# freshman97/LinTransUNet

Hardware: AMD Instinct MI355X
Metric: 128^3 CT patches/sec (fwd+bwd) (higher is better)
Workload: dtype bf16; 1 GPU; MaskTransUnet train step (fwd + 5-level loss + bwd), 128^3 single-channel patches, 2 per GPU, dropout 0.3, random-init weights; global_batch=2, parallelism=dp1, side_stream_concurrent=True, allreduce=none (1 rank)

## Files before the change

include/ltu_hip.h:

```cpp
#ifndef LTU_HIP_H
#define LTU_HIP_H

#include <stdint.h>

#ifdef __cplusplus
extern "C" {
#endif

typedef void* ltu_stream_t;

enum { LTU_F32 = 0, LTU_BF16 = 1 };
enum { LTU_OK = 0, LTU_E_DTYPE = -1, LTU_E_SHAPE = -2, LTU_E_ALIGN = -3, LTU_E_ARG = -4,
       LTU_E_COMM = -100  };
enum { LTU_ACT_NONE = 0, LTU_ACT_LRELU = 1 };

int ltu_version(void);
int ltu_build_flags(void);
int ltu_config_set(const char* name, int value, int clear);
int ltu_selftest_group_reduce(const float* x, float* sum, float* mx, int n, int G, ltu_stream_t s);
#ifdef LTU_EXPERIMENTS
int ltu_selftest_last_arriver(const float* x, float* part, float* out, unsigned* counter, float* sink, int nwg, int n,
                              int rows_per_chunk, int skew, int mode, ltu_stream_t s);
#endif

int ltu_window_embed(const float* x, void* y, int dtype, int B, int H, int W, int D, ltu_stream_t s);

int ltu_pack_conv_weight(const float* w, void* wf, void* wd, int Co, int Ci, int CoP, int CiP, int out_dtype, ltu_stream_t s);
int ltu_unpack_conv_wgrad(const float* dwf, float* dw, int Co, int Ci, int CiP, ltu_stream_t s);
int ltu_transpose_f32(const float* in, void* out, int R, int C, int ldo, int col_off, int out_dtype, ltu_stream_t s);
int ltu_cast_f32(const float* in, void* out, long long n, int out_dtype, ltu_stream_t s);
int ltu_weight_prep(const void* table, int n, int out_dtype, ltu_stream_t s);
#define LTU_WPREP_CHUNK 4096
int ltu_weight_prep_chunks(const void* table, const int* chunks, int nchunks, int out_dtype, ltu_stream_t s);

int ltu_linear_fwd(const void* a, int lda, const void* const* w, int nw, const float* const* bias, void* y, int ldy,
                   int M, int N, int K, int accumulate, int dtype, ltu_stream_t s);
int ltu_linear_gelu_fwd(const void* a, int lda, const void* w, const float* bias, void* u, void* h, int M, int N, int K, float p,
                        uint64_t seed, const uint64_t* step, int dtype, ltu_stream_t s);
int ltu_layer_tail_fwd(const void* a, const void* x, const void* wo, const void* w1, const void* w2, const float* bo,
                       const float* b1, const float* b2, const float* g1, const float* be1, const float* g2, const float* be2,
                       void* z1, void* t1, void* u, void* h, void* z2, void* y, float* stat1, float* stat2, long long M, int d,
                       float eps, float p, uint64_t seed1, uint64_t seedg, uint64_t seed2, const uint64_t* step, int u_mode,
                       const void* qkv, const float* ctx, float* qstat, int ntok, const void* wq_next, const float* bq0,
                       const float* bq1, const float* bq2, void* qkv_next, int dtype, ltu_stream_t s);

long long ltu_layer_tail_blocks(long long M);
int ltu_layer_tail_bwd(const void* dy, const void* dy2, const void* z2, const void* z1, const void* u, const float* stat2,
                       const float* stat1, const float* g2, const float* g1, const void* w2t, const void* w1t, const void* wot,
                       void* dr2, void* du, void* dr1, void* dz1, void* da, float* lnws2, float* lnws1, long long lnws_floats ,
                       long long M, int d, float p,
                       uint64_t seed1, uint64_t seedg, uint64_t seed2, const uint64_t* step, int u_mode, int dtype, ltu_stream_t s);

typedef struct ltu_reduce_job {
  const float* part;
  int nsplit, n, k, nseg;
  float* out[3];
  float* outb[3];
  int mode;
} ltu_reduce_job;
int ltu_reduce_batch(const ltu_reduce_job* jobs, int njobs, ltu_stream_t s);

long long ltu_wgrad_ws_floats(long long M, int N, int K);
int ltu_linear_wgrad(const void* g, int ldg, const void* a, int lda, float* const* dw, float* const* db, int nw, int M, int N,
                     int K, float* ws, long long ws_floats, ltu_reduce_job* defer, int dtype, ltu_stream_t s);
#define LTU_WGRAD_GROUP_MAX 32
typedef struct ltu_wgrad_job {
  const void* grad;
  const void* a;
  float* dw[3];
  float* db[3];
  int ldg, lda, nw, M, N, K;
} ltu_wgrad_job;
long long ltu_linear_wgrad_group_ws_floats(const ltu_wgrad_job* jobs, int njobs, int blocks);
int ltu_linear_wgrad_group(const ltu_wgrad_job* jobs, int njobs, int blocks, float* ws, long long ws_floats, int dtype, ltu_stream_t s);

long long ltu_upconv_wgrad_ws_floats(long long M, int Co, int Ci, int blocks);

int ltu_conv3d_fwd(const void* x0, const void* x1, const void* wf, const float* bias, void* y, int B, int Hi, int Wi,
                   int Di, int C0, int C1, int Co, int sh, int sw, int sd, int ups, float* ws, long long ws_floats, int dtype,
                   ltu_stream_t s);
long long ltu_conv3d_ws_floats(int B, int H, int W, int D, int C, int Co);
long long ltu_igemm_ws_floats(long long M, int N, int K);
int ltu_conv3d_pair_fwd(const void* x, const void* wf, const float* bias, void* y0, void* y1, int B, int H, int W, int D, int C,
                        int N0, int N1, float* ws, long long ws_floats, int dtype, ltu_stream_t s);
// ... 194 lines not shown
```

lintransunet_amd/_lib.py:

```python
import ctypes
import os
from ctypes import c_float, c_int, c_longlong, c_uint64, c_void_p

_HERE = os.path.dirname(os.path.abspath(__file__))
LIB_PATH = os.path.join(_HERE, os.environ.get('LTU_LIB', 'libltu_hip.so'))

P, I, L, F, U = c_void_p, c_int, c_longlong, c_float, c_uint64


class ReduceJob(ctypes.Structure):
    _fields_ = [('part', c_void_p), ('nsplit', c_int), ('n', c_int), ('k', c_int), ('nseg', c_int),
                ('out', c_void_p * 3), ('outb', c_void_p * 3), ('mode', c_int)]


class WgradJob(ctypes.Structure):
    _fields_ = [('grad', c_void_p), ('a', c_void_p), ('dw', c_void_p * 3), ('db', c_void_p * 3),
                ('ldg', c_int), ('lda', c_int), ('nw', c_int), ('M', c_int), ('N', c_int), ('K', c_int)]


WGRAD_GROUP_MAX = 32
CROP_ORIENT_MAX = 64
BLEND_ITEMS_MAX = 32
U8, I16 = 2, 3


SIGNATURES = {
    'ltu_version': [],
    'ltu_build_flags': [],
    'ltu_config_set': [ctypes.c_char_p, I, I],
    'ltu_selftest_group_reduce': [P, P, P, I, I, P],
    'ltu_window_embed': [P, P, I, I, I, I, I, P],
    'ltu_pack_conv_weight': [P, P, P, I, I, I, I, I, P],
    'ltu_unpack_conv_wgrad': [P, P, I, I, I, P],
    'ltu_transpose_f32': [P, P, I, I, I, I, I, P],
    'ltu_cast_f32': [P, P, L, I, P],
    'ltu_linear_fwd': [P, I, P, I, P, P, I, I, I, I, I, I, P],
    'ltu_wgrad_ws_floats': [L, I, I],
    'ltu_upconv_wgrad_ws_floats': [L, I, I, I],
    'ltu_linear_wgrad': [P, I, P, I, P, P, I, I, I, I, P, L, P, I, P],
    'ltu_layer_tail_fwd': [P, P, P, P, P, P, P, P, P, P, P, P, P, P, P, P, P, P, P, P, L, I, F, F, U, U, U, P, I, P, P, P, I, P, P, P, P, P, I, P],
    'ltu_layer_tail_blocks': [L],
    'ltu_layer_tail_bwd': [P, P, P, P, P, P, P, P, P, P, P, P, P, P, P, P, P, P, P, L, L, I, F, U, U, U, P, I, I, P],
    'ltu_reduce_batch': [P, I, P],
    'ltu_linear_wgrad_group_ws_floats': [P, I, I],
    'ltu_linear_wgrad_group': [P, I, I, P, L, I, P],
    'ltu_conv3d_fwd': [P, P, P, P, P, I, I, I, I, I, I, I, I, I, I, I, P, L, I, P],
    'ltu_conv3d_ws_floats': [I, I, I, I, I, I],
    'ltu_conv3d_pair_fwd': [P, P, P, P, P, I, I, I, I, I, I, I, P, L, I, P],
    'ltu_conv3d_pair_dgrad': [P, P, P, P, I, I, I, I, I, I, I, P, L, I, P],
    'ltu_conv3d_pair_wgrad': [P, P, P, P, P, P, P, I, I, I, I, I, I, I, I, I, I, P, L, I, P],
    'ltu_conv3d_dgrad': [P, P, P, P, I, I, I, I, I, I, I, I, I, I, P, L, I, P],
    'ltu_conv3d_wgrad': [P, P, P, P, P, I, I, I, I, I, I, I, I, I, I, I, I, I, P, L, I, P],
    'ltu_affine_sample': [P, P, P, I, I, I, I, P],
    'ltu_zoom_sample': [P, P, P, I, I, I, I, P],
    'ltu_adjust_contrast': [P, P, P, P, I, L, P],
    'ltu_linear_gelu_fwd': [P, I, P, P, P, P, I, I, I, F, U, P, I, P],
    'ltu_weight_prep': [P, I, I, P],
    'ltu_weight_prep_chunks': [P, P, I, I, P],
    'ltu_sumpool2': [P, P, I, I, I, I, I, I, P],
    'ltu_upconv_fwd': [P, P, P, P, I, I, I, I, I, I, I, P],
    'ltu_upconv_dgrad': [P, P, P, I, I, I, I, I, I, P, L, I, P],
    'ltu_igemm_ws_floats': [L, I, I],
    'ltu_upconv_wgrad': [P, P, P, P, P, I, I, P, L, I, I, I, I, I, I, I, I, P],
    'ltu_linattn_splits': [I, I],
    'ltu_linattn_ws_floats': [I, I, I],
    'ltu_linattn_fwd': [P, P, P, P, P, P, L, I, I, I, I, P],
    'ltu_linattn_ctx': [P, P, P, P, L, I, I, I, I, P],
    'ltu_linattn_bwd': [P, P, P, P, P, P, P, P, P, L, I, I, I, I, P],
    'ltu_window_gather': [P, P, P, I, I, I, I, I, I, I, I, I, I, P],
    'ltu_vote_accumulate': [P, P, P, P, I, I, I, I, I, I, I, I, P],
    'ltu_vote_finalize': [P, P, P, I, I, I, I, I, I, I, I, I, I, I, P],
    'ltu_window_gather_mirror': [P, P, P, I, I, I, I, I, I, I, I, I, I, I, P],
    'ltu_window_blend': [P, P, P, P, P, P, F, P, I, I, I, I, I, I, I, I, I, P],
    'ltu_keep_largest_component': [P, P, P, P, P, I, I, I, I, I, P],
    'ltu_seg_metrics': [P, P, P, P, I, I, I, I, L, F, P],
# ... 119 lines not shown
```

lintransunet_amd/csrc/misc.hip:

```cpp
#include <math.h>

#include "common.h"

#include <mutex>
#include <stdlib.h>

extern "C" int ltu_version(void) { return 4; }
extern "C" int ltu_build_flags(void) {
#ifdef LTU_EXPERIMENTS
  return 1;
#else
  return 0;
#endif
}

template <int G>
__global__ void selftest_reduce_kernel(const float* __restrict__ x, float* __restrict__ sum, float* __restrict__ mx, int n) {
  const int i = blockIdx.x * blockDim.x + threadIdx.x;
  const float v = i < n ? x[i] : 0.f;
  const float s = group_reduce<G, LtuAdd>(v), m = group_reduce<G, LtuMax>(v);
  if (i < n) { sum[i] = s; mx[i] = m; }
}
extern "C" int ltu_selftest_group_reduce(const float* x, float* sum, float* mx, int n, int G, ltu_stream_t s) {
  if (n <= 0 || n % 64) return LTU_E_SHAPE;
// ... 125 lines not shown
    const unsigned dr = stride % R, dc = stride / R;
    for (unsigned i = t0; i < t1; i += stride) {
      st1<TW>(dst + (size_t)c * d.p0 + d.p1 + r, d.src[(size_t)r * C + c]);
      r += dr; c += dc;
      if (r >= R) { r -= R; ++c; }
    }
  } else if (d.kind == 5 || d.kind == 6) {
    const unsigned CoP = (unsigned)d.p0, CiP = (unsigned)d.p1;
    const unsigned n = 64u * CoP * CiP;
    if (t1 > n) t1 = n;
    for (unsigned i = t0; i < t1; i += stride) {
      unsigned cls, sl, co, ci;
      if (d.kind == 5) { ci = i % CiP; const unsigned q = i / CiP; sl = q & 7; co = (q >> 3) % CoP; cls = (q >> 3) / CoP; }
      else { co = i % CoP; const unsigned q = i / CoP; const unsigned cs = q & 63; ci = q >> 6; cls = cs >> 3; sl = cs & 7; }
      float v = 0.f;
      if (co < (unsigned)d.R && ci < (unsigned)d.C) {
        int lo[3], hi[3];
        for (int a = 0; a < 3; ++a) {
          const int p = (cls >> (2 - a)) & 1, sa = (sl >> (2 - a)) & 1;
          if (p == 0) { lo[a] = sa == 0 ? 0 : 1; hi[a] = sa == 0 ? 0 : 2; }
          else { lo[a] = sa == 0 ? 0 : 2; hi[a] = sa == 0 ? 1 : 2; }
        }
        const float* w = d.src + ((size_t)co * d.C + ci) * 27;
        for (int th = lo[0]; th <= hi[0]; ++th)
          for (int tw = lo[1]; tw <= hi[1]; ++tw)
            for (int td = lo[2]; td <= hi[2]; ++td) v += w[(th * 3 + tw) * 3 + td];
      }
      st1<TW>(dst + i, v);
    }
  } else if (d.kind == 8 || d.kind == 9) {
    const unsigned n = (unsigned)d.R * (unsigned)d.C;
    if (t1 > n) t1 = n;
    const unsigned KS = (d.kind == 8 ? (unsigned)d.C : (unsigned)d.R) >> 4;
    for (unsigned i = t0; i < t1; i += stride) {
      const unsigned j = i & 7u, l = (i >> 3) & 63u, t = i >> 9;
      const unsigned ks = t % KS, ct = t / KS;
      const unsigned o = ct * 32u + (l & 31u), r = ks * 16u + 8u * (l >> 5) + j;
      const float v = d.kind == 8 ? d.src[(size_t)o * d.C + r] : d.src[(size_t)r * d.C + o];
      st1<TW>(dst + i, v);
    }
  } else if (d.kind == 7) {
    const unsigned stride_c = (unsigned)d.p0, CiP = (unsigned)d.p1, off = (unsigned)d.pad >> 16, cnt = (unsigned)d.pad & 0xffffu;
    const unsigned n = cnt * 27u * CiP;
    if (t1 > n) t1 = n;
    for (unsigned i = t0; i < t1; i += stride) {
      const unsigned co = i % cnt, q = i / cnt, t = q % 27u, ci = q / 27u;
      const float v = (co < (unsigned)d.R && ci < (unsigned)d.C) ? d.src[((size_t)co * d.C + ci) * 27 + t] : 0.f;
      st1<TW>(dst + ((size_t)ci * 27 + t) * stride_c + off + co, v);
    }
  } else {
    const unsigned CoP = (unsigned)d.p0, CiP = (unsigned)d.p1;
    const unsigned n = CoP * 27u * CiP;
    if (t1 > n) t1 = n;
    const unsigned R0 = d.kind == 2 ? CiP : CoP;
    unsigned x0 = t0 % R0, q = t0 / R0, x1 = q % 27u, x2 = q / 27u;
    const unsigned s0 = stride % R0, sq = stride / R0, s1 = sq % 27u, s2 = sq / 27u;
    for (unsigned i = t0; i < t1; i += stride) {
      const unsigned co = d.kind == 2 ? x2 : x0, ci = d.kind == 2 ? x0 : x2;
      const float v = (co < (unsigned)d.R && ci < (unsigned)d.C) ? d.src[((size_t)co * d.C + ci) * 27 + x1] : 0.f;
      st1<TW>(dst + i, v);
      x0 += s0; x1 += s1; x2 += s2;
      if (x0 >= R0) { x0 -= R0; ++x1; }
      if (x1 >= 27u) { x1 -= 27u; ++x2; }
    }
  }
}

template <typename TW>
__global__ void weight_prep_kernel(const WPrep* __restrict__ table) {
  const WPrep d = table[blockIdx.y];
  weight_prep_range<TW>(d, blockIdx.x * blockDim.x + threadIdx.x, 0x7fffffffu, gridDim.x * blockDim.x);
}
// ... 6 lines not shown
  return true;
}
__device__ __forceinline__ size_t wp8_load(const WPrep& d, unsigned i, float (&f)[8]) {
  const unsigned R = (unsigned)d.R, C = (unsigned)d.C;
  const bool src16 = (reinterpret_cast<uintptr_t>(d.src) & 15) == 0;
  size_t o = i;
  if (d.kind == 0) {
    if (src16) {
      const float4 a = *reinterpret_cast<const float4*>(d.src + i), b = *reinterpret_cast<const float4*>(d.src + i + 4);
      f[0] = a.x; f[1] = a.y; f[2] = a.z; f[3] = a.w; f[4] = b.x; f[5] = b.y; f[6] = b.z; f[7] = b.w;
    } else {
#pragma unroll
      for (int j = 0; j < 8; ++j) f[j] = d.src[i + j];
    }
  } else if (d.kind == 1) {
    const unsigned c = i / R, r = i - c * R;
#pragma unroll
    for (int j = 0; j < 8; ++j) f[j] = d.src[(size_t)(r + j) * C + c];
    o = (size_t)c * d.p0 + d.p1 + r;
  } else {
    const unsigned KS = (d.kind == 8 ? C : R) >> 4;
    const unsigned l = (i >> 3) & 63u, t = i >> 9;
    const unsigned ks = t % KS, ct = t / KS;
    const unsigned oo = ct * 32u + (l & 31u), r = ks * 16u + 8u * (l >> 5);
    if (d.kind == 8 && src16 && C % 4 == 0) {
      const float4 a = *reinterpret_cast<const float4*>(d.src + (size_t)oo * C + r), b = *reinterpret_cast<const float4*>(d.src + (size_t)oo * C + r + 4);
      f[0] = a.x; f[1] = a.y; f[2] = a.z; f[3] = a.w; f[4] = b.x; f[5] = b.y; f[6] = b.z; f[7] = b.w;
    } else if (d.kind == 8) {
#pragma unroll
      for (int j = 0; j < 8; ++j) f[j] = d.src[(size_t)oo * C + r + j];
    } else {
#pragma unroll
      for (int j = 0; j < 8; ++j) f[j] = d.src[(size_t)(r + j) * C + oo];
    }
  }
  return o;
}

template <typename TW, int WP_NC>
__global__ void __launch_bounds__(256) weight_prep_chunk_kernel(const WPrep* __restrict__ table, const int2* __restrict__ chunks, int nchunks) {
  constexpr int PER = LTU_WPREP_CHUNK / 8 / 256;
  static_assert(PER * 256 * 8 == LTU_WPREP_CHUNK, "chunk size");
  for (int c0 = blockIdx.x * WP_NC; c0 < nchunks; c0 += gridDim.x * WP_NC) {
    float f[WP_NC][PER][8];
    uint16_t* dp[WP_NC][PER];
#pragma unroll
    for (int k = 0; k < WP_NC; ++k) {
#pragma unroll
      for (int u = 0; u < PER; ++u) dp[k][u] = nullptr;
      if (c0 + k >= nchunks) continue;
      const int2 c = chunks[c0 + k];
      const WPrep d = table[c.x];
      const unsigned t0 = (unsigned)c.y * LTU_WPREP_CHUNK;
      if (!wp8_ok(d, (int)sizeof(TW))) {
        weight_prep_range<TW>(d, t0 + threadIdx.x, t0 + LTU_WPREP_CHUNK, blockDim.x);
        continue;
      }
      const unsigned n = (unsigned)d.R * (unsigned)d.C;
#pragma unroll
      for (int u = 0; u < PER; ++u) {
        const unsigned i = t0 + (threadIdx.x + u * 256u) * 8u;
        if (i < n) dp[k][u] = reinterpret_cast<uint16_t*>(d.dst) + wp8_load(d, i, f[k][u]);
      }
    }
#pragma unroll
    for (int k = 0; k < WP_NC; ++k)
// ... 74 lines not shown
```

lintransunet_amd/csrc/tlayer.hip:

```cpp
#include "common.h"

#define TL_ROWS 32
#ifndef TL_QDEPTH
#define TL_QDEPTH 8
#endif

struct TailArgs {
  const uint16_t* a;
  const uint16_t* x;
  const uint16_t* wo;
  const uint16_t* w1;
  const uint16_t* w2;
  const float* bo;
  const float* b1;
  const float* b2;
  const float* g1;
  const float* be1;
  const float* g2;
  const float* be2;
  uint16_t* z1;
  uint16_t* t1;
  uint16_t* u;
  uint16_t* h;
  uint16_t* z2;
// ... 348 lines not shown
    for (int i = tid; i < TL_ROWS * CPRQ; i += NTHR) {
      const int r = i / CPRQ, c = (i % CPRQ) * 8;
      if (row0 + r < ta.M) *reinterpret_cast<uint4*>(ta.qkv_next + (row0 + r) * (3 * D) + c) = *reinterpret_cast<const uint4*>(QB + r * LDQ + c);
    }
  }
}

struct TailBwdArgs {
  const uint16_t* dy;
  const uint16_t* dy2;
  const uint16_t* z2;
  const uint16_t* z1;
  const uint16_t* u;
  const float* stat2;
  const float* stat1;
  const float* g2;
  const float* g1;
  const uint16_t* w2t;
  const uint16_t* w1t;
  const uint16_t* wot;
  uint16_t* dr2;
  uint16_t* du;
  uint16_t* dr1;
  uint16_t* dz1;
  uint16_t* da;
  float* lnws2;
  float* lnws1;
  long long M;
  float p;
  uint64_t seed1, seedg, seed2;
  const uint64_t* step;
  int u_mode;
};

template <int D, int NTHR, bool G_LDS, bool G2_LDS, bool DZ_LDS, bool DZ_GLOBAL>
__device__ __forceinline__ void tl_layernorm_bwd(const uint16_t* gl_, const uint16_t* gl2_, const uint16_t* gg1, const uint16_t* gg2,
                                                 const uint16_t* __restrict__ zg, const float* __restrict__ stat,
                                                 const float* __restrict__ gamma, uint16_t* dzl, uint16_t* dzg, uint16_t* drl,
                                                 uint16_t* drg, float* __restrict__ lnws, float* red, int LD, long long row0,
                                                 long long M, const DropCfg& dc, int tid) {
  constexpr int E = D == 128 ? TL_LN_E128 : TL_LN_E256, Q = E / 4;
  constexpr int G = D / E, RPP = NTHR / G, NR = TL_ROWS / RPP;
  const int gl = tid % G, rgp = tid / G;
  float gmv[E], ag[E], ab[E];
#pragma unroll
  for (int q = 0; q < Q; ++q) {
    const float4 t = *reinterpret_cast<const float4*>(gamma + gl * E + 4 * q);
    gmv[4 * q] = t.x; gmv[4 * q + 1] = t.y; gmv[4 * q + 2] = t.z; gmv[4 * q + 3] = t.w;
  }
#pragma unroll
  for (int k = 0; k < E; ++k) { ag[k] = 0.f; ab[k] = 0.f; }
  uint2 zq[NR][Q], q1[NR][Q], q2[NR][Q];
  float2 st[NR];
#pragma unroll
  for (int i = 0; i < NR; ++i) {
    const long long row = row0 + rgp + i * RPP;
#pragma unroll
    for (int q = 0; q < Q; ++q) zq[i][q] = q1[i][q] = q2[i][q] = make_uint2(0u, 0u);
    st[i] = make_float2(0.f, 0.f);
    if (row < M) {
      ld_quads<Q>(zg + row * D + gl * E, zq[i]);
      if (gg1 != nullptr) ld_quads<Q>(gg1 + row * D + gl * E, q1[i]);
      if (gg2 != nullptr) ld_quads<Q>(gg2 + row * D + gl * E, q2[i]);
      st[i] = *reinterpret_cast<const float2*>(stat + row * 2);
    }
  }
// ... 30 lines not shown
      if (ok) { ab[k] += gv[k]; ag[k] += gv[k] * h[k]; }
      gg[k] = gv[k] * gmv[k];
      s1 += gg[k]; s2 += gg[k] * h[k];
    }
    const float m1 = group_sum<G>(s1) / (float)D, m2 = group_sum<G>(s2) / (float)D;
    uint2 dzq[Q], drq[Q];
#pragma unroll
    for (int q = 0; q < Q; ++q) {
      const float4 dz = make_float4(rstd * (gg[4 * q] - m1 - h[4 * q] * m2), rstd * (gg[4 * q + 1] - m1 - h[4 * q + 1] * m2),
                                    rstd * (gg[4 * q + 2] - m1 - h[4 * q + 2] * m2), rstd * (gg[4 * q + 3] - m1 - h[4 * q + 3] * m2));
      dzq[q] = pack_quad(dz.x, dz.y, dz.z, dz.w);
      const float4 dr = drop4(dc, (unsigned long long)(((row * D + gl * E) >> 2) + q), dz);
      drq[q] = pack_quad(dr.x, dr.y, dr.z, dr.w);
    }
    if constexpr (DZ_LDS) st_quads<Q>(dzl + r * LD + gl * E, dzq);
    st_quads<Q>(drl + r * LD + gl * E, drq);
    if (ok) {
      if constexpr (DZ_GLOBAL) st_quads<Q>(dzg + row * D + gl * E, dzq);
      st_quads<Q>(drg + row * D + gl * E, drq);
    }
  }
  float* dst = red + ((long long)rgp * D + gl * E) * 2;
#pragma unroll
  for (int k = 0; k < E; ++k) { dst[2 * k] = ag[k]; dst[2 * k + 1] = ab[k]; }
  __syncthreads();
  for (int i = tid; i < 2 * D; i += NTHR) {
    float acc = 0.f;
#pragma unroll
    for (int q = 0; q < RPP; ++q) acc += red[(long long)q * 2 * D + i];
    lnws[(long long)blockIdx.x * 2 * D + i] = acc;
  }
}

template <int D, int UMODE, int WPS, bool PRE_U>
__global__ void __launch_bounds__(D >= 256 ? 512 : 256, WPS) tail_bwd_kernel(const TailBwdArgs ta) {
  constexpr int LD = D + 8, LDH = 2 * D + 8;
  constexpr int NW = D >= 256 ? 8 : 4, NTHR = NW * 64;
  constexpr int NT1 = D / 32, NT2 = 2 * D / 32;
  static_assert(NT1 == NW && NT2 == 2 * NW, "one d-wide tile and two 2d-wide tiles per wave");
  constexpr int KS1 = D / 16, KS2 = 2 * D / 16;
  extern __shared__ __attribute__((aligned(16))) uint16_t smem[];
  uint16_t* RB = smem;
  uint16_t* ZB = RB + TL_ROWS * LD;
  uint16_t* UB = ZB + TL_ROWS * LD;
  float* red = reinterpret_cast<float*>(UB);
  static_assert((NTHR / (D / (D == 128 ? TL_LN_E128 : TL_LN_E256))) * 2 * D * sizeof(float) <= TL_ROWS * LDH * sizeof(uint16_t), "column-sum scratch fits in UB");
  const int tid = threadIdx.x, lane = tid & 63, wave = tid >> 6;
  const int li = lane & 31, lh = lane >> 5;
  const long long row0 = (long long)blockIdx.x * TL_ROWS;
  const DropCfg dc1 = make_drop(ta.p, ta.seed1, ta.step), dcg = make_drop(ta.p, ta.seedg, ta.step), dc2 = make_drop(ta.p, ta.seed2, ta.step);

  TlQueue<KS1> q1;
  TlQueue<KS2> q2;
  tl_layernorm_bwd<D, NTHR, false, false, true, false>(nullptr, nullptr, ta.dy, ta.dy2, ta.z2, ta.stat2, ta.g2, ZB, nullptr, RB, ta.dr2,
                                                      ta.lnws2, red, LD, row0, ta.M, dc2, tid);
  tl_issue<KS1>(ta.w2t, wave, lane, q1);
  constexpr int CPR2 = 2 * D / 8, NCH2 = TL_ROWS * CPR2 / NTHR;
  uint4 uch[PRE_U ? NCH2 : 1];
  if constexpr (PRE_U) {
#pragma unroll
    for (int j = 0; j < NCH2; ++j) {
      const int i = tid + j * NTHR, r = i / CPR2, c = (i % CPR2) * 8;
      uch[j] = make_uint4(0u, 0u, 0u, 0u);
      if (row0 + r < ta.M) uch[j] = *reinterpret_cast<const uint4*>(ta.u + (row0 + r) * (2 * D) + c);
    }
  }
  __builtin_amdgcn_sched_barrier(0);
  __syncthreads();
  f32x16 acc;
#pragma unroll
  for (int t = 0; t < 2; ++t) {
    const int ct = wave + t * NW;
    tl_run<KS1>(ta.w2t, ct, RB, LD, lane, q1, acc);
    if (t == 0) tl_issue<KS1>(ta.w2t, wave + NW, lane, q1);
    else tl_issue<KS2>(ta.w1t, wave, lane, q2);
#pragma unroll
    for (int q = 0; q < 4; ++q) {
      const int n = ct * 32 + 8 * q + 4 * lh;
      *reinterpret_cast<uint2*>(UB + li * LDH + n) = pack_quad(acc[4 * q], acc[4 * q + 1], acc[4 * q + 2], acc[4 * q + 3]);
    }
  }
  __syncthreads();
#pragma unroll
  for (int j = 0; j < NCH2; ++j) {
    const int i = tid + j * NTHR, r = i / CPR2, c = (i % CPR2) * 8;
    const long long rw = row0 + r;
    const uint4 dv = *reinterpret_cast<const uint4*>(UB + r * LDH + c);
    const float4 d0 = unpack_quad(make_uint2(dv.x, dv.y)), d1 = unpack_quad(make_uint2(dv.z, dv.w));
// ... 15 lines not shown
    }
    const uint4 dq = make_uint4(a0.x, a0.y, a1.x, a1.y);
    *reinterpret_cast<uint4*>(UB + r * LDH + c) = dq;
    if (rw < ta.M) *reinterpret_cast<uint4*>(ta.du + rw * (2 * D) + c) = dq;
  }
  __syncthreads();
  tl_run<KS2>(ta.w1t, wave, UB, LDH, lane, q2, acc);
  tl_issue<KS1>(ta.wot, wave, lane, q1);
#pragma unroll
  for (int q = 0; q < 4; ++q) {
    const int n = wave * 32 + 8 * q + 4 * lh;
    *reinterpret_cast<uint2*>(RB + li * LD + n) = pack_quad(acc[4 * q], acc[4 * q + 1], acc[4 * q + 2], acc[4 * q + 3]);
  }
  __syncthreads();
  tl_layernorm_bwd<D, NTHR, true, true, false, true>(RB, ZB, nullptr, nullptr, ta.z1, ta.stat1, ta.g1, nullptr, ta.dz1, RB, ta.dr1, ta.lnws1,
                                                    red, LD, row0, ta.M, dc1, tid);
  __syncthreads();
  tl_run<KS1>(ta.wot, wave, RB, LD, lane, q1, acc);
#pragma unroll
  for (int q = 0; q < 4; ++q) {
    const int n = wave * 32 + 8 * q + 4 * lh;
    *reinterpret_cast<uint2*>(ZB + li * LD + n) = pack_quad(acc[4 * q], acc[4 * q + 1], acc[4 * q + 2], acc[4 * q + 3]);
  }
  __syncthreads();
  {
    constexpr int CPR = D / 8;
    for (int i = tid; i < TL_ROWS * CPR; i += NTHR) {
      const int r = i / CPR, c = (i % CPR) * 8;
      if (row0 + r < ta.M) *reinterpret_cast<uint4*>(ta.da + (row0 + r) * D + c) = *reinterpret_cast<const uint4*>(ZB + r * LD + c);
    }
  }
}

extern "C" long long ltu_layer_tail_blocks(long long M) { return (M + TL_ROWS - 1) / TL_ROWS; }

extern "C" int ltu_layer_tail_bwd(const void* dy, const void* dy2, const void* z2, const void* z1, const void* u, const float* stat2,
                                  const float* stat1, const float* g2, const float* g1, const void* w2t, const void* w1t,
                                  const void* wot, void* dr2, void* du, void* dr1, void* dz1, void* da, float* lnws2, float* lnws1,
                                  long long lnws_floats, long long M, int d, float p, uint64_t seed1, uint64_t seedg, uint64_t seed2, const uint64_t* step,
                                  int u_mode, int dtype, ltu_stream_t s) {
  if (dtype != LTU_BF16) return LTU_E_DTYPE;
  if (d != 128 && d != 256) return LTU_E_SHAPE;
  if (u_mode != 0 && u_mode != 1) return LTU_E_ARG;
  if (M <= 0) return LTU_OK;
  if (lnws_floats < ltu_layer_tail_blocks(M) * 2 * d) return LTU_E_ARG;
  TailBwdArgs ta;
  ta.u_mode = u_mode;
  ta.dy = (const uint16_t*)dy; ta.dy2 = (const uint16_t*)dy2; ta.z2 = (const uint16_t*)z2; ta.z1 = (const uint16_t*)z1;
  ta.u = (const uint16_t*)u; ta.stat2 = stat2; ta.stat1 = stat1; ta.g2 = g2; ta.g1 = g1;
  ta.w2t = (const uint16_t*)w2t; ta.w1t = (const uint16_t*)w1t; ta.wot = (const uint16_t*)wot;
  ta.dr2 = (uint16_t*)dr2; ta.du = (uint16_t*)du; ta.dr1 = (uint16_t*)dr1; ta.dz1 = (uint16_t*)dz1; ta.da = (uint16_t*)da;
  ta.lnws2 = lnws2; ta.lnws1 = lnws1;
  ta.M = M; ta.p = p; ta.seed1 = seed1; ta.seedg = seedg; ta.seed2 = seed2; ta.step = step;
  const unsigned blocks = cdiv(M, TL_ROWS);
  const size_t lds = (size_t)TL_ROWS * (2 * (d + 8) + (2 * d + 8)) * sizeof(uint16_t);
  auto launch = [&](auto kern, unsigned threads) {
    static LtuDevOnce once;
    if (once.first()) ltu_dyn_lds(kern, 160 * 1024);
    hipLaunchKernelGGL(kern, dim3(blocks), dim3(threads), lds, (hipStream_t)s, ta);
  };
  if (d == 256) {
    if (ltu_knob("LTU_TAIL_BWD_PREU", 0)) { if (u_mode) launch(&tail_bwd_kernel<256, 1, 4, true>, 512); else launch(&tail_bwd_kernel<256, 0, 4, true>, 512); }
    else { if (u_mode) launch(&tail_bwd_kernel<256, 1, 4, false>, 512); else launch(&tail_bwd_kernel<256, 0, 4, false>, 512); }
  } else if (ltu_knob("LTU_TAIL_BWD_WPS", 4) == 3) {
    if (u_mode) launch(&tail_bwd_kernel<128, 1, 3, true>, 256); else launch(&tail_bwd_kernel<128, 0, 3, true>, 256);
  } else if (ltu_knob("LTU_TAIL_BWD_PREU", 1) == 0) {
    if (u_mode) launch(&tail_bwd_kernel<128, 1, 4, false>, 256); else launch(&tail_bwd_kernel<128, 0, 4, false>, 256);
  } else {
    if (u_mode) launch(&tail_bwd_kernel<128, 1, 4, true>, 256); else launch(&tail_bwd_kernel<128, 0, 4, true>, 256);
  }
  return ltu_check_launch();
}

extern "C" int ltu_layer_tail_fwd(const void* a, const void* x, const void* wo, const void* w1, const void* w2, const float* bo,
                                  const float* b1, const float* b2, const float* g1, const float* be1, const float* g2,
                                  const float* be2, void* z1, void* t1, void* u, void* h, void* z2, void* y, float* stat1,
                                  float* stat2, long long M, int d, float eps, float p, uint64_t seed1, uint64_t seedg,
                                  uint64_t seed2, const uint64_t* step, int u_mode, const void* qkv, const float* ctx, float* qstat,
                                  int ntok, const void* wq_next, const float* bq0, const float* bq1, const float* bq2,
                                  void* qkv_next, int dtype, ltu_stream_t s) {
  if (dtype != LTU_BF16) return LTU_E_DTYPE;
  if (d != 128 && d != 256) return LTU_E_SHAPE;
  if (u_mode != 0 && u_mode != 1) return LTU_E_ARG;
  if (qkv != nullptr && (ctx == nullptr || qstat == nullptr || ntok <= 0 || ntok % TL_ROWS || M % ntok)) return LTU_E_ARG;
  if (qkv_next != nullptr && (wq_next == nullptr || bq0 == nullptr || bq1 == nullptr || bq2 == nullptr)) return LTU_E_ARG;
  if (M <= 0) return LTU_OK;
// ... 39 lines not shown
```

lintransunet_amd/model.py:

```python
import os

import torch
import torch.nn as nn

from . import ops

HEAD_DIM = 32
N_LAYERS = 8


def _cl(t):
    return t.permute(0, 4, 1, 2, 3)


class _Group(nn.Module):
    """anonymous parameter container"""


def _transformer_layer(d):
    lay = _Group()
    lay.self_attn = _Group()
    lay.self_attn.linears = nn.ModuleList([nn.Linear(d, d) for _ in range(4)])
    lay.linear1 = nn.Linear(d, 2 * d)
    lay.linear2 = nn.Linear(2 * d, d)
# ... 57 lines not shown
        self.conv[id(conv)] = ops.UpConvPrep(wf, wd)

    def add_conv_pair(self, key, conv_a, conv_b, n1):
        wa, wb = conv_a.weight, conv_b.weight
        Ca, Ci = wa.shape[0], wa.shape[1]
        wf = torch.empty((Ca + n1, 27, Ci), device=self.device, dtype=self.dtype)
        wd = torch.empty((Ci, 27, Ca + n1), device=self.device, dtype=self.dtype)
        bias = torch.zeros(Ca + n1, device=self.device, dtype=torch.float32)
        self.raw.append((conv_a, conv_b, n1, wf, wd, bias))
        self.pair[key] = ops.PairPrep(wf, wd, bias, Ca, n1)

    def add_linear(self, key, weights, group=None, frag=False):
        N, K = weights[0].shape[0], weights[0].shape[1]
        if self.dtype == torch.float32:
            fw = list(weights)
        else:
            fw = []
            for w in weights:
                c = torch.empty((N, K), device=self.device, dtype=self.dtype)
                self.recs.append((w, c, 0, N, K, 0, 0))
                fw.append(c)
        wt = torch.empty((K, N * len(weights)), device=self.device, dtype=self.dtype)
        for i, w in enumerate(weights):
            self.recs.append((w, wt, 1, N, K, N * len(weights), i * N))
        fr = frT = None
        if frag and self.dtype == torch.bfloat16 and N % 32 == 0 and K % 32 == 0:
            nw = len(weights)
            fr = torch.empty(nw * N * K, device=self.device, dtype=self.dtype)
            for i, w in enumerate(weights):
                self.recs.append((w, fr[i * N * K:(i + 1) * N * K], 8, N, K, 0, 0))
            if nw == 1:
                frT = torch.empty(N * K, device=self.device, dtype=self.dtype)
                self.recs.append((weights[0], frT, 9, N, K, 0, 0))
        self.lin[key] = ops.LinPrep(fw, wt, group, fr, frT)

    def finalize(self):
        import numpy as np
        rows = [(src.data_ptr(), dst.data_ptr(), kind, R, C, p0, p1, 0) for src, dst, kind, R, C, p0, p1 in self.recs]
        for conv_a, conv_b, n1, wf, wd, bias in self.raw:
            rows += ops.pair_records(conv_a.weight, conv_a.bias, conv_b.weight, conv_b.bias, n1, wf, wd, bias)
        rec = np.zeros(len(rows), dtype=ops.WPREP_DTYPE)
        for i, r in enumerate(rows):
            rec[i] = r
        self.ptrs = [r[0] for r in rows]
        self.srcs = [src for src, *_ in self.recs] + [t for conv_a, conv_b, *_ in self.raw
                                                      for t in (conv_a.weight, conv_b.weight, conv_a.weight, conv_b.weight, conv_a.bias, conv_b.bias)]
        self.table = torch.from_numpy(rec.view(np.uint8).copy()).to(self.device)
        chunks = []
        for i, (_, _, kind, R, C, p0, p1, pad) in enumerate(rows):
            if kind in (0, 1, 4, 8, 9):
                n = R * C
            elif kind in (2, 3):
                n = p0 * 27 * p1
            elif kind == 7:
                n = (pad & 0xffff) * 27 * p1
            else:
                n = 64 * p0 * p1
            chunks += [(i, c) for c in range((n + WPREP_CHUNK - 1) // WPREP_CHUNK)]
        self.nchunks = len(chunks)
        self.chunks = torch.tensor(chunks, dtype=torch.int32).reshape(-1, 2).to(self.device)
        marks = list(getattr(self, 'marks', [])) + [len(rows)]
        self.bounds = [0] + [sum(1 for i, _ in chunks if i < m) for m in marks]

    def stale(self):
        return any(src.data_ptr() != p0 for src, p0 in zip(self.srcs, self.ptrs))

# ... 278 lines not shown
```

lintransunet_amd/ops.py:

```python
import contextlib
import ctypes
import threading

import torch

from . import _lib

F32, BF16 = 0, 1
ACT_NONE, ACT_LRELU = 0, 1
LRELU_SLOPE = 0.01
_c_void_p = ctypes.c_void_p


def _dt(t):
    if t.dtype == torch.float32:
        return F32
    if t.dtype == torch.bfloat16:
        return BF16
    raise TypeError(f'unsupported activation dtype {t.dtype}')


def _p(t):
    return 0 if t is None else t.data_ptr()

# ... 963 lines not shown
        g = g.contiguous()
        du = torch.empty_like(u)
        _lib.call('ltu_gelu_dropout_bwd', _p(g), _p(u), _p(du), u.numel(), float(p), seed, lc.step_ptr(), _dt(u), _s())
        return du, None, None


def gelu_dropout(u, p=0.0, seed=0):
    return _GeluDropout.apply(u, p, seed)


USE_LAYER_TAIL = _os.environ.get('LTU_NO_LAYER_TAIL', '') == ''
USE_LAYER_TAIL_BWD = _os.environ.get('LTU_NO_LAYER_TAIL_BWD', '') == ''
TAIL_MAX_TOKENS = int(_os.environ.get('LTU_TAIL_MAX_TOKENS', '1000000000'))


def _wgrad_now_or_group(lc, g, x, ws, bs, M, N, K):
    gw = [_grad_buf(w) for w in ws]
    gb = [_grad_buf(b) for b in bs]
    dws, dbs = [t for t, _ in gw], [t for t, _ in gb]
    if GROUP_WGRAD and all(f for _, f in gw) and all(f for _, f in gb):
        lc.wgrad_group_push(g, x, dws, dbs, M, N, K, False)
    else:
        wsb = _wgrad_ws(M, N, K, x)
        _lib.call('ltu_linear_wgrad', _p(g), N, _p(x), K, _ptr_array(dws), _ptr_array(dbs), len(ws), M, N, K,
                  _p(wsb), _n(wsb), 0, _dt(x), _s())
    return [_grad_done(w, t, f) for w, (t, f) in zip(ws, gw)], [_grad_done(b, t, f) for b, (t, f) in zip(bs, gb)]


FUSE_ATTN_APPLY = True
FUSE_ATTN_MAX_TOKENS = int(_os.environ.get('LTU_FUSE_ATTN_MAX_TOKENS', '1000000000'))
FUSE_NEXT_QKV = _os.environ.get('LTU_NO_FUSE_QKV', '') == ''
FUSE_QKV_MAX_TOKENS = int(_os.environ.get('LTU_FUSE_QKV_MAX_TOKENS', '50000'))
FUSE_QKV_MIN_TOKENS = int(_os.environ.get('LTU_FUSE_QKV_MIN_TOKENS', '0'))


class _LayerTail(torch.autograd.Function):

    @staticmethod
    def forward(ctx, a, x, wo, bo, w1, b1, w2, b2, g1, be1, g2, be2, preps, eps, p, seeds, fork, attn, nq0=None, nq1=None, nq2=None,
                nb0=None, nb1=None, nb2=None, nprep=None):
        lc = ctx.lc = current()
        _chk(a, 'a'); _chk(x, 'x')
        M, d = x.shape
        dev, dt = x.device, x.dtype
        po, p1, p2 = preps
        qkv = cx = colstats = qstat = None
        if attn is not None:
            B, N = attn
            qkv, H = a, d // 32
            nsplit = _lib.load().ltu_linattn_splits(B, N)
            cx = torch.empty((B * H, 32, 32), device=dev, dtype=torch.float32)
            colstats = torch.empty((B * H, 64), device=dev, dtype=torch.float32)
            qstat = torch.empty((M, H, 2), device=dev, dtype=torch.float32)
            ws = torch.empty(_lib.load().ltu_linattn_ws_floats(B, N, d), device=dev, dtype=torch.float32)
            _lib.call('ltu_linattn_ctx', _p(qkv), _p(cx), _p(colstats), _p(ws), _n(ws), B, N, d, _dt(qkv), _s())
            a = torch.empty((M, d), device=dev, dtype=dt)
        z1, t1, z2, y = (torch.empty((M, d), device=dev, dtype=dt) for _ in range(4))
        u, h = (torch.empty((M, 2 * d), device=dev, dtype=dt) for _ in range(2))
        stat1, stat2 = (torch.empty((M, 2), device=dev, dtype=torch.float32) for _ in range(2))
        qkv_next = torch.empty((M, 3 * d), device=dev, dtype=dt) if nprep is not None else None
        u_mode = 1 if (USE_LAYER_TAIL_BWD and po.fragT is not None and p1.fragT is not None and p2.fragT is not None) else 0
        _lib.call('ltu_layer_tail_fwd', _p(a), _p(x), _p(po.frag), _p(p1.frag), _p(p2.frag), _p(bo), _p(b1), _p(b2), _p(g1), _p(be1),
                  _p(g2), _p(be2), _p(z1), _p(t1), _p(u), _p(h), _p(z2), _p(y), _p(stat1), _p(stat2), M, d, float(eps), float(p),
                  seeds[0], seeds[1], seeds[2], lc.step_ptr(), u_mode, _p(qkv), _p(cx), _p(qstat), attn[1] if attn else 0,
                  _p(nprep.frag) if nprep is not None else 0, _p(nb0), _p(nb1), _p(nb2), _p(qkv_next), _dt(a), _s())
        ctx.save_for_backward(a, z1, stat1, t1, u, h, z2, stat2, y if nprep is not None else None)
        ctx.params = (wo, bo, w1, b1, w2, b2, g1, be1, g2, be2)
        ctx.cfg = (preps, p, seeds)
        ctx.u_mode = u_mode
        ctx.attn = None if attn is None else (attn, qkv, cx, colstats, qstat)
        ctx.nxt = None if nprep is None else ((nq0, nq1, nq2), (nb0, nb1, nb2), nprep)
        if nprep is not None:
            return y, qkv_next
        return (y, y.view_as(y)) if fork else y

    @staticmethod
    def backward(ctx, g, g2=None):
        lc = ctx.lc
        a, z1, stat1, t1, u, h, z2, stat2, y = ctx.saved_tensors
        wo, bo, w1, b1, w2, b2, gm1, be1, gm2, be2 = ctx.params
        (po, p1, p2), p, seeds = ctx.cfg
        M, d = a.shape
        dev, dt = a.device, _dt(a)
        nxt_grads = (None,) * 7
        if ctx.nxt is not None:
            (nws, nbs, nprep), gq = ctx.nxt, g2
            g2 = None
            if gq is not None:
                gq = gq.contiguous()
                g2 = torch.empty((M, d), device=dev, dtype=a.dtype)
                _lib.call('ltu_linear_fwd', _p(gq), 3 * d, _ptr_array([nprep.wt]), 1, _ptr_array([None]), _p(g2), d, M, d, 3 * d, 0, dt, _s())
                gw = [_grad_buf(w) for w in nws]
                gb = [_grad_buf(b) for b in nbs]
                dws, dbs = [t for t, _ in gw], [t for t, _ in gb]
                if GROUP_WGRAD and all(f for _, f in gw) and all(f for _, f in gb):
                    lc.wgrad_group_push(gq, y, dws, dbs, M, 3 * d, d, True)
                else:
                    wsq = _wgrad_ws(M, 3 * d, d, y)
                    _lib.call('ltu_linear_wgrad', _p(gq), 3 * d, _p(y), d, _ptr_array(dws), _ptr_array(dbs), 3, M, 3 * d, d,
                              _p(wsq), _n(wsq), 0, dt, _s())
                nxt_grads = tuple(_grad_done(w, t, f) for w, (t, f) in zip(nws, gw)) + \
                    tuple(_grad_done(b, t, f) for b, (t, f) in zip(nbs, gb)) + (None,)
        if g is None:
            g, g2 = g2, None
        g = g.contiguous()
        if g2 is not None:
            g2 = g2.contiguous()

        def ln_bwd(gy, gy2, z, stat, gamma, beta, seed):
            dz = torch.empty_like(z)
            dr = torch.empty_like(z) if p > 0 else dz
            dg, fg = _grad_buf(gamma)
            db, fb = _grad_buf(beta)
            job, ws = None, lc.norm_ws(dev)
            if fg and fb:
                job = _defer_job()
                ws = torch.empty(2048 * 2 * d, device=dev, dtype=torch.float32)
            _lib.call('ltu_layernorm_bwd', _p(gy), _p(gy2), _p(z), _p(stat), _p(gamma), _p(dz), _p(dr), _p(dg), _p(db), _p(ws), _n(ws),
                      ctypes.addressof(job) if job is not None else 0, M, d, float(p), seed, lc.step_ptr(), dt, _s())
            if job is not None:
                lc.defer_push(job, ws)
            return dz, dr, _grad_done(gamma, dg, fg), _grad_done(beta, db, fb)

        def dgrad(gy, prep, w, N, K):
            wt = prep.wt if prep is not None else _w_transposed([w], N, K, a.dtype)
            dx = torch.empty((M, K), device=dev, dtype=a.dtype)
            _lib.call('ltu_linear_fwd', _p(gy), N, _ptr_array([wt]), 1, _ptr_array([None]), _p(dx), K, M, K, N, 0, dt, _s())
            return dx

        if ctx.u_mode == 1:
            dr2, dr1, dz1, da = (torch.empty_like(a) for _ in range(4))
            du = torch.empty_like(u)
            nblk = _lib.load().ltu_layer_tail_blocks(M)
            lnws = torch.empty((2, nblk, 2 * d), device=dev, dtype=torch.float32)
            _lib.call('ltu_layer_tail_bwd', _p(g), _p(g2), _p(z2), _p(z1), _p(u), _p(stat2), _p(stat1), _p(gm2), _p(gm1), _p(p2.fragT),
                      _p(p1.fragT), _p(po.fragT), _p(dr2), _p(du), _p(dr1), _p(dz1), _p(da), _p(lnws[0]), _p(lnws[1]), _n(lnws[0]), M, d, float(p),
                      seeds[0], seeds[1], seeds[2], lc.step_ptr(), 1, dt, _s())
            outs = []
            for k, (gamma, beta) in enumerate(((gm2, be2), (gm1, be1))):
                dg, fg = _grad_buf(gamma)
                db, fb = _grad_buf(beta)
                job = _defer_job()
                job.part, job.nsplit, job.n, job.k, job.nseg, job.mode = lnws[k].data_ptr(), nblk, 2 * d, 1, 1, 1
                job.out[0], job.out[1] = dg.data_ptr(), db.data_ptr()
                if fg and fb:
                    lc.defer_push(job, lnws)
                else:
                    _lib.call('ltu_reduce_batch', ctypes.addressof(job), 1, _s())
                outs.append((_grad_done(gamma, dg, fg), _grad_done(beta, db, fb)))
            (dgm2, dbe2), (dgm1, dbe1) = outs
            (dw2,), (db2,) = _wgrad_now_or_group(lc, dr2, h, [w2], [b2], M, d, 2 * d)
            (dw1,), (db1,) = _wgrad_now_or_group(lc, du, t1, [w1], [b1], M, 2 * d, d)
            (dwo,), (dbo,) = _wgrad_now_or_group(lc, dr1, a, [wo], [bo], M, d, d)
            return (_LayerTail._attn_bwd(ctx, da), dz1, dwo, dbo, dw1, db1, dw2, db2, dgm1, dbe1, dgm2, dbe2, None, None, None, None, None, None) + (nxt_grads if ctx.nxt is not None else ())
        dz2, dr2, dgm2, dbe2 = ln_bwd(g, g2, z2, stat2, gm2, be2, seeds[2])
        dh = dgrad(dr2, p2, w2, d, 2 * d)
        (dw2,), (db2,) = _wgrad_now_or_group(lc, dr2, h, [w2], [b2], M, d, 2 * d)
        du = torch.empty_like(u)
        _lib.call('ltu_gelu_dropout_bwd', _p(dh), _p(u), _p(du), u.numel(), float(p), seeds[1], lc.step_ptr(), dt, _s())
        dt1 = dgrad(du, p1, w1, 2 * d, d)
        (dw1,), (db1,) = _wgrad_now_or_group(lc, du, t1, [w1], [b1], M, 2 * d, d)
        dz1, dr1, dgm1, dbe1 = ln_bwd(dt1, dz2, z1, stat1, gm1, be1, seeds[0])
        da = dgrad(dr1, po, wo, d, d)
        (dwo,), (dbo,) = _wgrad_now_or_group(lc, dr1, a, [wo], [bo], M, d, d)
        return (_LayerTail._attn_bwd(ctx, da), dz1, dwo, dbo, dw1, db1, dw2, db2, dgm1, dbe1, dgm2, dbe2, None, None, None, None, None, None) + (nxt_grads if ctx.nxt is not None else ())

    @staticmethod
    def _attn_bwd(ctx, da):
        if ctx.attn is None:
            return da
# ... 409 lines not shown
```

Baseline: 164.8 patches/s.

## Fuse next-layer QKV dgrad GEMM into the layer-tail backward kernel

In the layer-tail backward, the gradient flowing back from the next layer's fused QKV projection used to be computed by a separate linear GEMM writing a d-wide buffer, which the tail kernel then read as dy2. A new kernel variant loads the dqkv tile into LDS, multiplies it by a stacked transposed QKV weight fragment, and feeds the result directly into the layernorm backward. This removes one GEMM launch and a global write/read of the M×d intermediate. To support it, weight prep now packs the three Q/K/V weights into one stacked fragment buffer. The trade-off is extra LDS and register pressure in the tail kernel, and the path only covers d=256 with bf16 and u_mode 1.

```diff
diff --git a/include/ltu_hip.h b/include/ltu_hip.h
--- a/include/ltu_hip.h
+++ b/include/ltu_hip.h
@@ -50,6 +50,11 @@
                        void* dr2, void* du, void* dr1, void* dz1, void* da, float* lnws2, float* lnws1, long long lnws_floats ,
                        long long M, int d, float p,
                        uint64_t seed1, uint64_t seedg, uint64_t seed2, const uint64_t* step, int u_mode, int dtype, ltu_stream_t s);
+int ltu_layer_tail_bwd_qkv(const void* dy, const void* dqkv, const void* wqkvt, const void* z2, const void* z1, const void* u,
+                           const float* stat2, const float* stat1, const float* g2, const float* g1, const void* w2t, const void* w1t,
+                           const void* wot, void* dr2, void* du, void* dr1, void* dz1, void* da, float* colsum2, float* colsum1,
+                           long long colsum_floats , long long M, int d, float p, uint64_t seed1, uint64_t seedg,
+                           uint64_t seed2, const uint64_t* step, int u_mode, int dtype, ltu_stream_t s);
 
 typedef struct ltu_reduce_job {
   const float* part;
diff --git a/lintransunet_amd/_lib.py b/lintransunet_amd/_lib.py
--- a/lintransunet_amd/_lib.py
+++ b/lintransunet_amd/_lib.py
@@ -41,6 +41,7 @@
     'ltu_layer_tail_fwd': [P, P, P, P, P, P, P, P, P, P, P, P, P, P, P, P, P, P, P, P, L, I, F, F, U, U, U, P, I, P, P, P, I, P, P, P, P, P, I, P],
     'ltu_layer_tail_blocks': [L],
     'ltu_layer_tail_bwd': [P, P, P, P, P, P, P, P, P, P, P, P, P, P, P, P, P, P, P, L, L, I, F, U, U, U, P, I, I, P],
+    'ltu_layer_tail_bwd_qkv': [P, P, P, P, P, P, P, P, P, P, P, P, P, P, P, P, P, P, P, P, L, L, I, F, U, U, U, P, I, I, P],
     'ltu_reduce_batch': [P, I, P],
     'ltu_linear_wgrad_group_ws_floats': [P, I, I],
     'ltu_linear_wgrad_group': [P, I, I, P, L, I, P],
diff --git a/lintransunet_amd/csrc/misc.hip b/lintransunet_amd/csrc/misc.hip
--- a/lintransunet_amd/csrc/misc.hip
+++ b/lintransunet_amd/csrc/misc.hip
@@ -181,12 +181,14 @@
     const unsigned n = (unsigned)d.R * (unsigned)d.C;
     if (t1 > n) t1 = n;
     const unsigned KS = (d.kind == 8 ? (unsigned)d.C : (unsigned)d.R) >> 4;
+    const bool stack = d.kind == 9 && d.p0 > 0;
+    const unsigned KT = stack ? (unsigned)d.p0 >> 4 : KS, k0 = stack ? (unsigned)d.p1 >> 4 : 0u;
     for (unsigned i = t0; i < t1; i += stride) {
       const unsigned j = i & 7u, l = (i >> 3) & 63u, t = i >> 9;
       const unsigned ks = t % KS, ct = t / KS;
       const unsigned o = ct * 32u + (l & 31u), r = ks * 16u + 8u * (l >> 5) + j;
       const float v = d.kind == 8 ? d.src[(size_t)o * d.C + r] : d.src[(size_t)r * d.C + o];
-      st1<TW>(dst + i, v);
+      st1<TW>(dst + (stack ? ((size_t)(ct * KT + ks + k0) * 64u + l) * 8u + j : (size_t)i), v);
     }
   } else if (d.kind == 7) {
     const unsigned stride_c = (unsigned)d.p0, CiP = (unsigned)d.p1, off = (unsigned)d.pad >> 16, cnt = (unsigned)d.pad & 0xffffu;
@@ -259,6 +261,7 @@
     } else {
 #pragma unroll
       for (int j = 0; j < 8; ++j) f[j] = d.src[(size_t)(r + j) * C + oo];
+      if (d.p0 > 0) o = ((size_t)(ct * ((unsigned)d.p0 >> 4) + ks + ((unsigned)d.p1 >> 4)) * 64u + l) * 8u;
     }
   }
   return o;
diff --git a/lintransunet_amd/csrc/tlayer.hip b/lintransunet_amd/csrc/tlayer.hip
--- a/lintransunet_amd/csrc/tlayer.hip
+++ b/lintransunet_amd/csrc/tlayer.hip
@@ -404,6 +404,10 @@
   const uint64_t* step;
   int u_mode;
 };
+struct TailBwdQkvArgs : TailBwdArgs {
+  const uint16_t* dqkv;
+  const uint16_t* wqt;
+};
 
 template <int D, int NTHR, bool G_LDS, bool G2_LDS, bool DZ_LDS, bool DZ_GLOBAL>
 __device__ __forceinline__ void tl_layernorm_bwd(const uint16_t* gl_, const uint16_t* gl2_, const uint16_t* gg1, const uint16_t* gg2,
@@ -500,8 +504,8 @@
   }
 }
 
-template <int D, int UMODE, int WPS, bool PRE_U>
-__global__ void __launch_bounds__(D >= 256 ? 512 : 256, WPS) tail_bwd_kernel(const TailBwdArgs ta) {
+template <int D, int UMODE, int WPS, bool PRE_U, bool QKVG, typename Args>
+__device__ __forceinline__ void tail_bwd_body(const Args ta) {
   constexpr int LD = D + 8, LDH = 2 * D + 8;
   constexpr int NW = D >= 256 ? 8 : 4, NTHR = NW * 64;
   constexpr int NT1 = D / 32, NT2 = 2 * D / 32;
@@ -520,8 +524,39 @@
 
   TlQueue<KS1> q1;
   TlQueue<KS2> q2;
+  if constexpr (QKVG) {
+    constexpr int LDQ = 3 * D + 8, KSQ = 3 * D / 16, CPRQ = 3 * D / 8, NCHQ = TL_ROWS * CPRQ / NTHR;
+    static_assert(LDQ <= LD + LDH && TL_ROWS * CPRQ % NTHR == 0, "the dqkv tile fits in ZB + UB");
+    uint16_t* QB = ZB;
+    TlQueue<KSQ> qq;
+    tl_issue<KSQ>(ta.wqt, wave, lane, qq);
+    uint4 ch[NCHQ];
+#pragma unroll
+    for (int j = 0; j < NCHQ; ++j) {
+      const int i = tid + j * NTHR, r = i / CPRQ, c = (i % CPRQ) * 8;
+      ch[j] = make_uint4(0u, 0u, 0u, 0u);
+      if (row0 + r < ta.M) ch[j] = *reinterpret_cast<const uint4*>(ta.dqkv + (row0 + r) * (3 * D) + c);
+    }
+#pragma unroll
+    for (int j = 0; j < NCHQ; ++j) {
+      const int i = tid + j * NTHR, r = i / CPRQ, c = (i % CPRQ) * 8;
+      *reinterpret_cast<uint4*>(QB + r * LDQ + c) = ch[j];
+    }
+    __syncthreads();
+    f32x16 accq;
+    tl_run<KSQ>(ta.wqt, wave, QB, LDQ, lane, qq, accq);
+#pragma unroll
+    for (int q = 0; q < 4; ++q) {
+      const int n = wave * 32 + 8 * q + 4 * lh;
+      *reinterpret_cast<uint2*>(RB + li * LD + n) = pack_quad(accq[4 * q], accq[4 * q + 1], accq[4 * q + 2], accq[4 * q + 3]);
+    }
+    __syncthreads();
+    tl_layernorm_bwd<D, NTHR, true, false, true, false>(RB, nullptr, ta.dy, nullptr, ta.z2, ta.stat2, ta.g2, ZB, nullptr, RB, ta.dr2,
+                                                       ta.lnws2, red, LD, row0, ta.M, dc2, tid);
+  } else {
   tl_layernorm_bwd<D, NTHR, false, false, true, false>(nullptr, nullptr, ta.dy, ta.dy2, ta.z2, ta.stat2, ta.g2, ZB, nullptr, RB, ta.dr2,
                                                       ta.lnws2, red, LD, row0, ta.M, dc2, tid);
+  }
   tl_issue<KS1>(ta.w2t, wave, lane, q1);
   constexpr int CPR2 = 2 * D / 8, NCH2 = TL_ROWS * CPR2 / NTHR;
   uint4 uch[PRE_U ? NCH2 : 1];
@@ -603,7 +638,53 @@
   }
 }
 
+template <int D, int UMODE, int WPS, bool PRE_U>
+__global__ void __launch_bounds__(D >= 256 ? 512 : 256, WPS) tail_bwd_kernel(const TailBwdArgs ta) {
+  tail_bwd_body<D, UMODE, WPS, PRE_U, false>(ta);
+}
+
+template <int D, int UMODE, int WPS, bool PRE_U>
+__global__ void __launch_bounds__(D >= 256 ? 512 : 256, WPS) tail_bwd_qkv_kernel(const TailBwdQkvArgs ta) {
+  tail_bwd_body<D, UMODE, WPS, PRE_U, true>(ta);
+}
+
 extern "C" long long ltu_layer_tail_blocks(long long M) { return (M + TL_ROWS - 1) / TL_ROWS; }
+
+static TailBwdArgs tail_bwd_args(const void* dy, const void* dy2, const void* z2, const void* z1, const void* u, const float* stat2,
+                                 const float* stat1, const float* g2, const float* g1, const void* w2t, const void* w1t,
+                                 const void* wot, void* dr2, void* du, void* dr1, void* dz1, void* da, float* lnws2, float* lnws1,
+                                 long long M, float p, uint64_t seed1, uint64_t seedg, uint64_t seed2, const uint64_t* step, int u_mode) {
+  TailBwdArgs ta;
+  ta.u_mode = u_mode;
+  ta.dy = (const uint16_t*)dy; ta.dy2 = (const uint16_t*)dy2; ta.z2 = (const uint16_t*)z2; ta.z1 = (const uint16_t*)z1;
+  ta.u = (const uint16_t*)u; ta.stat2 = stat2; ta.stat1 = stat1; ta.g2 = g2; ta.g1 = g1;
+  ta.w2t = (const uint16_t*)w2t; ta.w1t = (const uint16_t*)w1t; ta.wot = (const uint16_t*)wot;
+  ta.dr2 = (uint16_t*)dr2; ta.du = (uint16_t*)du; ta.dr1 = (uint16_t*)dr1; ta.dz1 = (uint16_t*)dz1; ta.da = (uint16_t*)da;
+  ta.lnws2 = lnws2; ta.lnws1 = lnws1;
+  ta.M = M; ta.p = p; ta.seed1 = seed1; ta.seedg = seedg; ta.seed2 = seed2; ta.step = step;
+  return ta;
+}
+
+extern "C" int ltu_layer_tail_bwd_qkv(const void* dy, const void* dqkv, const void* wqkvt, const void* z2, const void* z1, const void* u,
+                                      const float* stat2, const float* stat1, const float* g2, const float* g1, const void* w2t,
+                                      const void* w1t, const void* wot, void* dr2, void* du, void* dr1, void* dz1, void* da,
+                                      float* lnws2, float* lnws1, long long lnws_floats, long long M, int d, float p, uint64_t seed1,
+                                      uint64_t seedg, uint64_t seed2, const uint64_t* step, int u_mode, int dtype, ltu_stream_t s) {
+  if (dtype != LTU_BF16) return LTU_E_DTYPE;
+  if (d != 256) return LTU_E_SHAPE;
+  if (u_mode != 1 || dqkv == nullptr || wqkvt == nullptr) return LTU_E_ARG;
+  if (M <= 0) return LTU_OK;
+  if (lnws_floats < ltu_layer_tail_blocks(M) * 2 * d) return LTU_E_ARG;
+  TailBwdQkvArgs ta;
+  static_cast<TailBwdArgs&>(ta) = tail_bwd_args(dy, nullptr, z2, z1, u, stat2, stat1, g2, g1, w2t, w1t, wot, dr2, du, dr1, dz1, da, lnws2, lnws1, M, p,
+                                                seed1, seedg, seed2, step, u_mode);
+  ta.dqkv = (const uint16_t*)dqkv; ta.wqt = (const uint16_t*)wqkvt;
+  const size_t lds = (size_t)TL_ROWS * (2 * (d + 8) + (2 * d + 8)) * sizeof(uint16_t);
+  static LtuDevOnce once;
+  if (once.first()) ltu_dyn_lds(&tail_bwd_qkv_kernel<256, 1, 4, false>, 160 * 1024);
+  hipLaunchKernelGGL((tail_bwd_qkv_kernel<256, 1, 4, false>), dim3(cdiv(M, TL_ROWS)), dim3(512), lds, (hipStream_t)s, ta);
+  return ltu_check_launch();
+}
 
 extern "C" int ltu_layer_tail_bwd(const void* dy, const void* dy2, const void* z2, const void* z1, const void* u, const float* stat2,
                                   const float* stat1, const float* g2, const float* g1, const void* w2t, const void* w1t,
@@ -615,14 +696,8 @@
   if (u_mode != 0 && u_mode != 1) return LTU_E_ARG;
   if (M <= 0) return LTU_OK;
   if (lnws_floats < ltu_layer_tail_blocks(M) * 2 * d) return LTU_E_ARG;
-  TailBwdArgs ta;
-  ta.u_mode = u_mode;
-  ta.dy = (const uint16_t*)dy; ta.dy2 = (const uint16_t*)dy2; ta.z2 = (const uint16_t*)z2; ta.z1 = (const uint16_t*)z1;
-  ta.u = (const uint16_t*)u; ta.stat2 = stat2; ta.stat1 = stat1; ta.g2 = g2; ta.g1 = g1;
-  ta.w2t = (const uint16_t*)w2t; ta.w1t = (const uint16_t*)w1t; ta.wot = (const uint16_t*)wot;
-  ta.dr2 = (uint16_t*)dr2; ta.du = (uint16_t*)du; ta.dr1 = (uint16_t*)dr1; ta.dz1 = (uint16_t*)dz1; ta.da = (uint16_t*)da;
-  ta.lnws2 = lnws2; ta.lnws1 = lnws1;
-  ta.M = M; ta.p = p; ta.seed1 = seed1; ta.seedg = seedg; ta.seed2 = seed2; ta.step = step;
+  const TailBwdArgs ta = tail_bwd_args(dy, dy2, z2, z1, u, stat2, stat1, g2, g1, w2t, w1t, wot, dr2, du, dr1, dz1, da, lnws2, lnws1, M, p,
+                                       seed1, seedg, seed2, step, u_mode);
   const unsigned blocks = cdiv(M, TL_ROWS);
   const size_t lds = (size_t)TL_ROWS * (2 * (d + 8) + (2 * d + 8)) * sizeof(uint16_t);
   auto launch = [&](auto kern, unsigned threads) {
diff --git a/lintransunet_amd/model.py b/lintransunet_amd/model.py
--- a/lintransunet_amd/model.py
+++ b/lintransunet_amd/model.py
@@ -113,6 +113,10 @@
             if nw == 1:
                 frT = torch.empty(N * K, device=self.device, dtype=self.dtype)
                 self.recs.append((weights[0], frT, 9, N, K, 0, 0))
+            else:
+                frT = torch.empty(nw * N * K, device=self.device, dtype=self.dtype)
+                for i, w in enumerate(weights):
+                    self.recs.append((w, frT, 9, N, K, nw * N, i * N))
         self.lin[key] = ops.LinPrep(fw, wt, group, fr, frT)
 
     def finalize(self):
diff --git a/lintransunet_amd/ops.py b/lintransunet_amd/ops.py
--- a/lintransunet_amd/ops.py
+++ b/lintransunet_amd/ops.py
@@ -1019,6 +1019,7 @@
 FUSE_NEXT_QKV = _os.environ.get('LTU_NO_FUSE_QKV', '') == ''
 FUSE_QKV_MAX_TOKENS = int(_os.environ.get('LTU_FUSE_QKV_MAX_TOKENS', '50000'))
 FUSE_QKV_MIN_TOKENS = int(_os.environ.get('LTU_FUSE_QKV_MIN_TOKENS', '0'))
+FUSE_QKV_BWD = _os.environ.get('LTU_NO_FUSE_QKV_BWD', '') == ''
 
 
 class _LayerTail(torch.autograd.Function):
@@ -1070,13 +1071,17 @@
         M, d = a.shape
         dev, dt = a.device, _dt(a)
         nxt_grads = (None,) * 7
+        gq_fused = None
         if ctx.nxt is not None:
             (nws, nbs, nprep), gq = ctx.nxt, g2
             g2 = None
             if gq is not None:
                 gq = gq.contiguous()
-                g2 = torch.empty((M, d), device=dev, dtype=a.dtype)
-                _lib.call('ltu_linear_fwd', _p(gq), 3 * d, _ptr_array([nprep.wt]), 1, _ptr_array([None]), _p(g2), d, M, d, 3 * d, 0, dt, _s())
+                if FUSE_QKV_BWD and g is not None and d == 256 and ctx.u_mode == 1 and nprep.fragT is not None:
+                    gq_fused = gq
+                else:
+                    g2 = torch.empty((M, d), device=dev, dtype=a.dtype)
+                    _lib.call('ltu_linear_fwd', _p(gq), 3 * d, _ptr_array([nprep.wt]), 1, _ptr_array([None]), _p(g2), d, M, d, 3 * d, 0, dt, _s())
                 gw = [_grad_buf(w) for w in nws]
                 gb = [_grad_buf(b) for b in nbs]
                 dws, dbs = [t for t, _ in gw], [t for t, _ in gb]
@@ -1120,9 +1125,14 @@
             du = torch.empty_like(u)
             nblk = _lib.load().ltu_layer_tail_blocks(M)
             lnws = torch.empty((2, nblk, 2 * d), device=dev, dtype=torch.float32)
-            _lib.call('ltu_layer_tail_bwd', _p(g), _p(g2), _p(z2), _p(z1), _p(u), _p(stat2), _p(stat1), _p(gm2), _p(gm1), _p(p2.fragT),
-                      _p(p1.fragT), _p(po.fragT), _p(dr2), _p(du), _p(dr1), _p(dz1), _p(da), _p(lnws[0]), _p(lnws[1]), _n(lnws[0]), M, d, float(p),
-                      seeds[0], seeds[1], seeds[2], lc.step_ptr(), 1, dt, _s())
+            if gq_fused is not None:
+                _lib.call('ltu_layer_tail_bwd_qkv', _p(g), _p(gq_fused), _p(nprep.fragT), _p(z2), _p(z1), _p(u), _p(stat2), _p(stat1), _p(gm2),
+                          _p(gm1), _p(p2.fragT), _p(p1.fragT), _p(po.fragT), _p(dr2), _p(du), _p(dr1), _p(dz1), _p(da), _p(lnws[0]), _p(lnws[1]),
+                          _n(lnws[0]), M, d, float(p), seeds[0], seeds[1], seeds[2], lc.step_ptr(), 1, dt, _s())
+            else:
+                _lib.call('ltu_layer_tail_bwd', _p(g), _p(g2), _p(z2), _p(z1), _p(u), _p(stat2), _p(stat1), _p(gm2), _p(gm1), _p(p2.fragT),
+                          _p(p1.fragT), _p(po.fragT), _p(dr2), _p(du), _p(dr1), _p(dz1), _p(da), _p(lnws[0]), _p(lnws[1]), _n(lnws[0]), M, d, float(p),
+                          seeds[0], seeds[1], seeds[2], lc.step_ptr(), 1, dt, _s())
             outs = []
             for k, (gamma, beta) in enumerate(((gm2, be2), (gm1, be1))):
                 dg, fg = _grad_buf(gamma)
```

Result: no change. 166.2 patches/s, median of 6 (+0.8%).
